# jhamrick/gaussian_processes

Measured on AMD Instinct MI355X. Metric: GP fit+predict wall-clock (kernel build + Cholesky + solve + log_lh + posterior mean), lower is better.
Workload: dtype f64; 1 GPU; N=65536 d=32 RBF(GaussianKernel) f64, m=1000 test points, h=1 w=0.5*sqrt(d) s=1; N=65536, d=32, m=1000, parallelism=1 GPU

## Files before the change

gaussian_processes_amd/_lib.py:

```python
import ctypes
import os
from ctypes import (POINTER, c_char_p, c_double, c_float, c_int, c_int64, c_size_t,
                    c_uint64, c_void_p)

import numpy as np

_HERE = os.path.dirname(os.path.abspath(__file__))
LIB_PATH = os.path.join(_HERE, "libgpx.so")

OK = 0
ERR_ARG, ERR_HIP, ERR_NO_DEVICE, ERR_NOMEM, ERR_UNSUPPORTED, ERR_INTERNAL = -1, -2, -3, -4, -5, -6
(ROUTE_TRSV_OPS, ROUTE_TRSV_STEPS, ROUTE_PANEL_RES, ROUTE_PANEL_CHAIN, ROUTE_FIT_RIDE, ROUTE_FIT_TWO_SOLVES,
 ROUTE_GEMM_FAST, ROUTE_GEMM_GENERIC, ROUTE_SYRK_EXACT, ROUTE_SYRK_PATCH, ROUTE_MG_BCAST_ONE, ROUTE_MG_BCAST_SAG,
 ROUTE_FIT_OPS_AHEAD, ROUTE_TRSM_OPS, ROUTE_POTRF_PAIR, ROUTE_VAR_CHUNK, ROUTE_LOO_CHUNK, ROUTE_TRSM_L_OPS,
 ROUTE_GRAD_CHUNK, ROUTE_EXTEND, ROUTE_SAMPLE, ROUTE_KAPPLY_FUSED, ROUTE_KAPPLY_GEMM, ROUTE_PATHS_GRAD_CHUNK,
 ROUTE_REMOVE, ROUTE_SPARSE_CHUNK) = range(26)
PROF_RANDN, PROF_RFF, PROF_KAPPLY, PROF_KAPPLY_GRAD, PROF_CHOL_DELETE, PROF_SPARSE_GRAM, PROF_SPARSE_GRAD = 14, 15, 16, 17, 18, 19, 20
F64, F32 = 0, 1
KERNEL_GAUSSIAN, KERNEL_PERIODIC, KERNEL_GAUSSIAN_ARD = 0, 1, 2
ARD_MAX_D = 64
FULL, LOWER = 0, 1
(K, DK_DH, DK_DW, DK_DP, D2K_DHDH, D2K_DHDW, D2K_DHDP, D2K_DWDW, D2K_DWDP, D2K_DPDP) = range(10)
MIN_LOG = -705.6238298100243

MEMBER_BY_NAME = {
    "K": K, "dK_dh": DK_DH, "dK_dw": DK_DW, "dK_dp": DK_DP,
    "d2K_dhdh": D2K_DHDH, "d2K_dhdw": D2K_DHDW, "d2K_dwdh": D2K_DHDW,
    "d2K_dhdp": D2K_DHDP, "d2K_dpdh": D2K_DHDP, "d2K_dwdw": D2K_DWDW,
    "d2K_dwdp": D2K_DWDP, "d2K_dpdw": D2K_DWDP, "d2K_dpdp": D2K_DPDP,
}

MG_ID_BYTES = 128
MG_BCAST_FN = ctypes.CFUNCTYPE(c_int, c_void_p, c_void_p, c_size_t, c_int, c_void_p)
MG_ALLREDUCE_FN = ctypes.CFUNCTYPE(c_int, c_void_p, c_void_p, c_size_t, c_int, c_int, c_void_p)

c_double_p = POINTER(c_double)
c_int_p = POINTER(c_int)

_SIGNATURES = {
    "gpx_version": (c_int, []),
    "gpx_last_error": (c_char_p, []),
    "gpx_device_count": (c_int, [c_int_p]),
    "gpx_set_device": (c_int, [c_int]),
    "gpx_get_device": (c_int, [c_int_p]),
    "gpx_device_info": (c_int, [c_int, c_char_p, c_size_t, c_int_p, c_int_p, POINTER(c_uint64)]),
    "gpx_malloc": (c_int, [POINTER(c_void_p), c_size_t]),
    "gpx_free": (c_int, [c_void_p]),
    "gpx_mem_info": (c_int, [ctypes.POINTER(c_size_t), ctypes.POINTER(c_size_t)]),
    "gpx_memcpy_h2d": (c_int, [c_void_p, c_void_p, c_size_t, c_void_p]),
# ... 316 lines not shown
```

gaussian_processes_amd/csrc/gpx_common.h:

```cpp
#pragma once
#include <hip/hip_runtime.h>
#include <stdint.h>
#include <stdio.h>
#include <stdlib.h>
#include <string.h>
#include <math.h>
#include <vector>

#include "../../include/gpx.h"
#include "gpx_tune.h"

namespace gpx {

void set_error(const char *fmt, ...);
int  hip_fail(hipError_t e, const char *what, const char *file, int line);
int  ensure_device();

#define GPX_HIP(call)                                                        \
    do {                                                                     \
        hipError_t e__ = (call);                                             \
        if (e__ != hipSuccess) return gpx::hip_fail(e__, #call, __FILE__, __LINE__); \
    } while (0)

#define GPX_TRY(call)                                                        \
    do {                                                                     \
        int rc__ = (call);                                                   \
        if (rc__ != GPX_OK) return rc__;                                     \
    } while (0)

#define GPX_ARG(cond, msg)                                                   \
    do {                                                                     \
        if (!(cond)) { gpx::set_error("%s: %s", __func__, msg); return GPX_ERR_ARG; } \
    } while (0)

#define GPX_LAUNCH_CHECK()                                                   \
    do {                                                                     \
        hipError_t e__ = hipGetLastError();                                  \
        if (e__ != hipSuccess) return gpx::hip_fail(e__, "kernel launch", __FILE__, __LINE__); \
    } while (0)


enum Route { RT_TRSV_OPS = 0, RT_TRSV_STEPS = 1, RT_PANEL_RES = 2, RT_PANEL_CHAIN = 3, RT_FIT_RIDE = 4,
             RT_FIT_TWO_SOLVES = 5, RT_GEMM_FAST = 6, RT_GEMM_GENERIC = 7, RT_SYRK_EXACT = 8, RT_SYRK_PATCH = 9,
             RT_MG_BCAST_ONE = 10, RT_MG_BCAST_SAG = 11, RT_FIT_OPS_AHEAD = 12, RT_TRSM_OPS = 13, RT_POTRF_PAIR = 14, RT_VAR_CHUNK = 15, RT_LOO_CHUNK = 16,
             RT_TRSM_L_OPS = 17, RT_GRAD_CHUNK = 18, RT_EXTEND = 19, RT_SAMPLE = 20, RT_KAPPLY_FUSED = 21, RT_KAPPLY_GEMM = 22, RT_PATHS_GRAD_CHUNK = 23, RT_REMOVE = 24, RT_SPARSE_CHUNK = 25, RT_COUNT = 26 };
void route_hit(int route);

int check_internal_info(int info);

static inline hipStream_t S(void *s) { return (hipStream_t)s; }
static inline size_t esize(int dtype) { return dtype == GPX_F64 ? 8 : 4; }
static inline int64_t round_up(int64_t v, int64_t m) { return (v + m - 1) / m * m; }
static inline int64_t cdiv(int64_t a, int64_t b) { return (a + b - 1) / b; }

static inline int order(hipEvent_t e, hipStream_t from, hipStream_t to)
{
    GPX_HIP(hipEventRecord(e, from));
    GPX_HIP(hipStreamWaitEvent(to, e, 0));
    return GPX_OK;
}
struct EventPool {
    std::vector<hipEvent_t> ev; size_t next = 0;
    int reserve(size_t count)
    {
        while (ev.size() < count) {
            hipEvent_t x;
            GPX_HIP(hipEventCreateWithFlags(&x, hipEventDisableTiming));
            ev.push_back(x);
        }
        return GPX_OK;
    }
    int get(hipEvent_t *e) { GPX_TRY(reserve(next + 1)); *e = ev[next++]; return GPX_OK; }
    void rewind() { next = 0; }
    void destroy() { for (hipEvent_t e : ev) (void)hipEventDestroy(e); ev.clear(); next = 0; }
    int order(hipStream_t from, hipStream_t to) { hipEvent_t e; GPX_TRY(get(&e)); return gpx::order(e, from, to); }
};

enum ProfClass { PC_KMAT = 0, PC_GEMM = 1, PC_POTRF_DIAG = 2, PC_TRSM_ROWS = 3, PC_TRSV = 4,
// ... 61 lines not shown
int syrk_bc(int dtype, int64_t n, int64_t row_begin, void *Cloc, int64_t ldc, int64_t cl0, int64_t cl1,
            const void *Pb, int64_t ldp, int64_t k0, int64_t kb, int64_t nb, int P, int rank,
            hipStream_t st, const int *abort_flag = nullptr, const Batch *bt = nullptr);
struct PanelHints { bool idle_chip = false; int leaf_force = 0; };
struct PotrfHook { int (*fn)(void *user, int64_t cols_done, hipEvent_t panel_done); void *user; };
int potrf_panel(int dtype, void *A, int64_t lda, int64_t n, int64_t r0, int64_t c0, int64_t kb,
                int *info_dev, hipStream_t st, const Batch *bt = nullptr, int64_t kpre = 0,
                hipEvent_t done = nullptr, PanelHints hints = {});
int potrf(int dtype, void *A, int64_t n, int64_t lda, int *info_dev, hipStream_t st, const Batch *bt = nullptr,
          int64_t xrows = 0,
          bool may_block = false,
          const PotrfHook *hook = nullptr);
int potrf_panel_res(int dtype, void *A, int64_t lda, int64_t n, int64_t r0, int64_t c0, int64_t kb, int *info_dev,
                    hipStream_t st, const Batch *bt = nullptr, int64_t kpre = 0, hipEvent_t done = nullptr, PanelHints hints = {});
int64_t panel_res_max();
hipStream_t potrf_side_stream();
bool kernel_values_finite(int kernel, const double *p, double s, int dtype);
bool panel_res_fold(int64_t rows, int64_t kpre, int64_t kb, size_t es, int64_t lda, const void *base);
constexpr int TRSV_OPS_BLOCK = 512;
static inline int64_t trsv_ops_nblocks(int64_t n) { return n / TRSV_OPS_BLOCK; }
static inline bool trsv_ops_whole_blocks(int64_t n) { return n >= TRSV_OPS_BLOCK && n % TRSV_OPS_BLOCK == 0; }
struct TrsvOps {
    GrowBuf mem;
    bool valid = false;
    int64_t built = 0;
    void invalidate() { valid = false; built = 0; }
    static TrsvOps view(void *p, size_t bytes) { TrsvOps o; o.mem.p = p; o.mem.bytes = bytes; return o; }
};
int trsv_ops_build(int dtype, const void *L, int64_t n, int64_t ldl, TrsvOps *ops, hipStream_t st);
bool trsv_ops_ahead_ok(int dtype, const void *L, int64_t n, int64_t ldl);
bool trsm_ops_ok(int dtype, const void *L, int64_t n, int64_t ldl);
size_t trsv_ops_bytes(int dtype, int64_t n);
int trsv_ops_build_upto(int dtype, const void *L, int64_t n, int64_t ldl, TrsvOps *ops, int64_t kend, hipStream_t st);
int trsv_lower(int dtype, const void *L, int64_t n, int64_t ldl, void *b, void *x, int transpose,
               hipStream_t st, const Batch *bt = nullptr,
               TrsvOps *ops = nullptr);
int trsm_right_lt(int dtype, const void *L, int64_t n, int64_t ldl, void *X, int64_t m, int64_t ldx,
                  hipStream_t st, int x_upper = 0, TrsvOps *ops = nullptr,
                  int64_t c0 = 0);
int trsm_right_l(int dtype, const void *L, int64_t n, int64_t ldl, void *X, int64_t m, int64_t ldx, hipStream_t st,
                 TrsvOps *ops = nullptr);
int pred_grad(int dtype, int kernel, const void *xo, int64_t m, const void *x, int64_t n, int d, const double *params,
              const void *alpha, const void *B, int64_t ldb, double scale, const double *col_div, double *out_dev, hipStream_t st);
int inv_from_factor(int dtype, const void *L, int64_t n, int64_t ldl, void *X, void *W, int tri, hipStream_t st,
                    TrsvOps *ops, int count = 1, int64_t sL = 0, void *group_ops = nullptr);
int logdet_chol(int dtype, const void *L, int64_t n, int64_t ldl, double *out_dev, hipStream_t st, int count = 1,
                int64_t sL = 0, int64_t so = 0);
int dot(int dtype, const void *a, const void *b, int64_t n, double *out_dev, hipStream_t st, int count = 1,
        int64_t sa = 0, int64_t sb = 0, int64_t so = 0);
int diag_sum(int dtype, const void *A, int64_t n, int64_t lda, double *out_dev, hipStream_t st);
int transpose(int dtype, const void *src, int64_t lds, int64_t rows, int64_t cols, void *dst, int64_t ldd, int mirror, hipStream_t st);
int tril(int dtype, void *A, int64_t n, int64_t lda, hipStream_t st);
int var_rows(int dtype, int kernel, const void *X, int64_t rows, int64_t n, int64_t ldx, const void *xo, int d,
             const double *params, const double *kdiag_dev, int accumulate, double *out_dev, hipStream_t st);
int var_finish(int dtype, int kernel, const void *xo, int d, const double *params, const double *acc_dev, int64_t rows,
               double *out_dev, hipStream_t st);
int eye_rows(int dtype, void *X, int64_t rows, int64_t ld, int64_t c0, int64_t cz, hipStream_t st);
int loo_rows(int dtype, const void *X, int64_t rows, int64_t n, int64_t ldx, int64_t c0, const void *y, const void *alpha,
             double *kii, double *mean, double *var, double *logp, hipStream_t st);
int loo_points(int dtype, const double *kii, const void *y, const void *alpha, int64_t n, double *mean, double *var, double *logp,
               hipStream_t st);
int sum_f64(const double *a, int64_t n, double *out_dev, hipStream_t st);
int copy_lower(int dtype, const void *src, int64_t lds, void *dst, int64_t ldd, int64_t n, hipStream_t st);
int schur_lower(int dtype, const void *B, int64_t k, int64_t n, int64_t ldb, void *S, int64_t lds, hipStream_t st);
int sum_slices_lower(int dtype, const void *P, int64_t ldp, int64_t sP, int slices, int64_t n, const void *minus_from, void *out, int64_t ldo,
                     hipStream_t st);
// ... 45 lines not shown
```

gaussian_processes_amd/csrc/gpx_gp.hip:

```cpp
#include "gpx_small.h"
#include <cmath>
#include <vector>

#include "gpx_gp_internal.h"

namespace gpx {

static int copy_rows(void *dst, int64_t ldd, const void *src, int64_t lds, int64_t rows, int64_t cols, hipMemcpyKind kind, hipStream_t st)
{
    if (rows == 1) GPX_HIP(hipMemcpyAsync(dst, src, (size_t)cols * 8, kind, st));
    else GPX_HIP(hipMemcpy2DAsync(dst, (size_t)ldd * 8, src, (size_t)lds * 8, (size_t)cols * 8, (size_t)rows, kind, st));
    return GPX_OK;
}

int upload_f64(int dtype, void *dst, int64_t ldd, const double *src, int64_t lds, int64_t rows, int64_t cols, hipStream_t st, DevBuf *stage)
{
    if (rows <= 0 || cols <= 0) return GPX_OK;
    if (dtype == GPX_F64) {
        GPX_TRY(copy_rows(dst, ldd, src, lds, rows, cols, hipMemcpyHostToDevice, st));
    } else {
        DevBuf mine;
        if (!stage) stage = &mine;
        if (!stage->p) GPX_TRY(stage->alloc((size_t)rows * cols * 8));
        GPX_TRY(copy_rows(stage->p, cols, src, lds, rows, cols, hipMemcpyHostToDevice, st));
// ... 37 lines not shown
    return scale_points(g->dtype, g->x, g->n, g->d, g->params + 1, g->xs, g->st);
}

static int upload_points(gpx_gp *g, void *dst, const double *xo, int64_t m)
{
    GPX_TRY(upload_f64(g->dtype, dst, m * g->d, xo, m * g->d, 1, m * g->d, g->st));
    if (g->kernel == GPX_KERNEL_GAUSSIAN_ARD) GPX_TRY(scale_points(g->dtype, dst, m, g->d, g->params + 1, dst, g->st));
    return GPX_OK;
}

int gp_read_scal(gpx_gp *g, GpScal *host)
{
    GPX_HIP(hipMemcpyAsync(host, g->scal, sizeof(GpScal), hipMemcpyDeviceToHost, g->st));
    GPX_HIP(hipStreamSynchronize(g->st));
    return check_internal_info(host->info);
}

int gp_need_factor(gpx_gp *g, const char *what_for)
{
    GpScal sc;
    GPX_TRY(gp_read_scal(g, &sc));
    if (sc.info != 0) { set_error("Kxx is not positive definite (info = %d): there is no factor %s", sc.info, what_for); return GPX_ERR_ARG; }
    return GPX_OK;
}

int check_internal_info(int info)
{
    if (info >= 0) return GPX_OK;
    set_error("internal failure inside the factorisation (info = %d: a hand-off between workgroups of the resident "
              "panel kernel timed out); the factor is not valid -- this is NOT a statement about the matrix", info);
    return GPX_ERR_INTERNAL;
}

int gp_finish_fit(gpx_gp *g, bool rhs_is_row_n, int *info)
{
    const size_t es = esize(g->dtype);
    hipStream_t st = g->st;
    if (rhs_is_row_n) {
        GPX_TRY(trsv_lower(g->dtype, g->A, g->n, g->lda, (char *)g->A + (size_t)g->n * g->lda * es, g->alpha, 1, st, nullptr, &g->ops));
    } else {
        GPX_HIP(hipMemcpyAsync(g->t0, g->y, (size_t)g->n * es, hipMemcpyDeviceToDevice, st));
        GPX_TRY(trsv_lower(g->dtype, g->A, g->n, g->lda, g->t0, g->t1, 0, st, nullptr, &g->ops));
        GPX_TRY(trsv_lower(g->dtype, g->A, g->n, g->lda, g->t1, g->alpha, 1, st, nullptr, &g->ops));
    }
    GPX_HIP(hipEventRecord(g->ev[3], st));
    GPX_TRY(logdet_chol(g->dtype, g->A, g->n, g->lda, &g->scal->logdet, st));
    GPX_TRY(dot(g->dtype, g->y, g->alpha, g->n, &g->scal->yta, st));
    GPX_HIP(hipEventRecord(g->ev[4], st));
    g->fitted = true;
    if (info) {
        GPX_HIP(hipMemcpyAsync(info, &g->scal->info, sizeof(int), hipMemcpyDeviceToHost, st));
        GPX_HIP(hipStreamSynchronize(st));
        GPX_TRY(check_internal_info(*info));
    }
    return GPX_OK;
}

template <typename T>
__global__ void nonfinite_kernel(const T *__restrict__ v, int64_t n, int *__restrict__ flag)
{
    bool bad = false;
    for (int64_t i = (int64_t)blockIdx.x * blockDim.x + threadIdx.x; i < n; i += (int64_t)gridDim.x * blockDim.x)
        bad = bad || !isfinite(v[i]);
    if (__any(bad) && (threadIdx.x & 63) == 0) atomicOr(flag, 1);
}

int gp_scan_finite(gpx_gp *g)
{
    int *flags = &g->scal->x_bad;
    GPX_HIP(hipMemsetAsync(flags, 0, 2 * sizeof(int), g->st));
    const int64_t nx = g->n * g->d, ny = g->n;
    const unsigned bx = (unsigned)std::min<int64_t>(cdiv(nx, 256), 1024), by = (unsigned)std::min<int64_t>(cdiv(ny, 256), 1024);
// ... 203 lines not shown
    return gp_scan_finite(g);
}

int gpx_gp_set_params(gpx_gp_t *g, const double *params, double s)
{
    GP_ENTER(g);
    GPX_ARG(g && params, "NULL argument");
    GPX_ARG(!(s < 0), "invalid value for s");
    for (int i = 0; i < g->nparams; ++i) g->params[i] = params[i];
    g->s = s;
    g->have_params = true; g->have_K = false; gp_unfit(g);
    return gp_rescale(g);
}

int gpx_gp_get_params(gpx_gp_t *g, double *params, int cap, int *count)
{
    GP_ENTER(g);
    GPX_ARG(g->have_params, "no kernel parameters in the handle");
    GPX_ARG(cap >= 0 && (cap == 0 || params), "bad arguments");
    if (count) *count = g->nparams;
    for (int i = 0; i < g->nparams && i < cap; ++i) params[i] = g->params[i];
    return GPX_OK;
}

int gpx_gp_set_K(gpx_gp_t *g, const double *Kxx, int64_t ld)
{
    GP_ENTER(g);
    GPX_ARG(g && Kxx && ld >= g->n, "bad arguments");
    GPX_TRY(upload_f64(g->dtype, g->A, g->lda, Kxx, ld, g->n, g->n, g->st));
    g->have_K = true; gp_unfit(g);
    return GPX_OK;
}

struct OpsAhead { gpx_gp *g; int64_t group, last; };
static int ops_ahead_step(void *user, int64_t cols_done, hipEvent_t panel_done)
{
    OpsAhead *o = (OpsAhead *)user;
    gpx_gp *g = o->g;
    const int64_t ready = std::min(trsv_ops_nblocks(cols_done), o->last);
    if (ready - g->ops.built < o->group) return GPX_OK;
    GPX_HIP(hipStreamWaitEvent(g->st_ops, panel_done, 0));
    return trsv_ops_build_upto(g->dtype, g->A, g->n, g->lda, &g->ops, ready, g->st_ops);
}

int gpx_gp_fit(gpx_gp_t *g, int *info)
{
    GP_ENTER(g);
    GPX_ARG(g, "gp is NULL");
    GPX_ARG(g->have_data && (g->have_params || g->have_K),
            "set_data and set_params (or set_K) must be called before fit");
    const GpView v = gp_view(g);
    if (!g->have_K && (!g->x_finite || !kernel_values_finite(v.kernel, v.params, g->s, g->dtype))) {
        set_error("%s (%s)", NONFINITE_MSG, g->x_finite ? "kernel parameters or s" : "x");
        return GPX_ERR_ARG;
    }
    const size_t es = esize(g->dtype);
    hipStream_t st = g->st;
    GPX_HIP(hipEventRecord(g->ev[0], st));
    if (!g->have_K)
        GPX_TRY(kmat(g->dtype, v.kernel, GPX_K, v.x, g->n, v.x, g->n, g->d, v.params, g->s * g->s,
                     GPX_LOWER, g->A, g->lda, st));
    g->have_K = false;
    g->have_kii = false;
    GPX_HIP(hipEventRecord(g->ev[1], st));
    const int64_t ride_max = tune().fit_ride_max;
    const bool ride = g->n <= ride_max;
    route_hit(ride ? RT_FIT_RIDE : RT_FIT_TWO_SOLVES);
    if (ride) GPX_HIP(hipMemcpyAsync((char *)g->A + (size_t)g->n * g->lda * es, g->y, (size_t)g->n * es, hipMemcpyDeviceToDevice, st));
    g->ops.invalidate();
    const bool ahead = tune().fit_ops_ahead != 0 && g->n >= tune().fit_ops_ahead_min &&
                       trsv_ops_ahead_ok(g->dtype, g->A, g->n, g->lda);
    const int64_t nfull = trsv_ops_nblocks(g->n), tail = tune().fit_ops_tail;
    const int64_t group = std::max<int64_t>(1, std::min(nfull, nfull - tail));
    OpsAhead oa = {g, group, std::max<int64_t>(0, nfull - tail)};
    PotrfHook hook = {ops_ahead_step, &oa};
    if (ahead) {
        if (!g->st_ops) {
            int least = 0, greatest = 0;
            GPX_HIP(hipDeviceGetStreamPriorityRange(&least, &greatest));
            GPX_HIP(hipStreamCreateWithPriority(&g->st_ops, hipStreamNonBlocking, least));
            GPX_HIP(hipEventCreateWithFlags(&g->ev_ops, hipEventDisableTiming));
        }
        GPX_TRY(g->ops.mem.reserve(trsv_ops_bytes(g->dtype, g->n), st));
        GPX_TRY(order(g->ev_ops, st, g->st_ops));
    }
    GPX_TRY(potrf(g->dtype, g->A, g->n, g->lda, &g->scal->info, st, nullptr, ride ? 1 : 0, true, ahead ? &hook : nullptr));
    if (ahead) {
        GPX_TRY(order(g->ev_ops, g->st_ops, st));
        if (g->ops.built > 0) route_hit(RT_FIT_OPS_AHEAD);
    }
    GPX_HIP(hipEventRecord(g->ev[2], st));
    return gp_finish_fit(g, ride, info);
}

static int gp_scalars(gpx_gp_t *g, double *logdet, double *yta, int *info)
{
    GP_ENTER(g);
    GPX_ARG(g && g->fitted, "gp is not fitted");
    GpScal sc;
    GPX_TRY(gp_read_scal(g, &sc));
    if (logdet) *logdet = sc.logdet;
    if (yta) *yta = sc.yta;
    if (info) *info = sc.info;
    return GPX_OK;
}

int gpx_gp_log_lh(gpx_gp_t *g, double *log_lh)
{
    GPX_ARG(log_lh, "log_lh is NULL");
    GPX_ARG(g, "gp is NULL");
    GP_NEED_FINITE_Y(g);
    double logdet, yta; int info;
    GPX_TRY(gp_scalars(g, &logdet, &yta, &info));
    if (info != 0 || !(logdet >= GPX_MIN_LOG)) { *log_lh = -INFINITY; return GPX_OK; }
    const double data_fit = -0.5 * yta;
    const double complexity_penalty = -0.5 * logdet;
    const double constant = -0.5 * (double)g->n * log(2 * M_PI);
    *log_lh = data_fit + complexity_penalty + constant;
    return GPX_OK;
}

int gpx_gp_logdet(gpx_gp_t *g, double *logdet)
{
    GPX_ARG(logdet, "logdet is NULL");
    return gp_scalars(g, logdet, nullptr, nullptr);
// ... 727 lines not shown
```

gaussian_processes_amd/csrc/gpx_gp_internal.h:

```cpp
#pragma once
#include "gpx_common.h"
#include <cstddef>

struct GpScal {
    double logdet;
    double yta;
    int x_bad, y_bad;
    int info;
    int pad;
};
static_assert(sizeof(GpScal) == 32 && offsetof(GpScal, x_bad) == 16 && offsetof(GpScal, info) == 24, "GpScal layout");

struct gpx_gp {
    int device;
    int dtype, kernel, d, nparams;
    int64_t n, lda;
    void *x, *y, *A, *alpha, *t0, *t1;
    void *xs;
    GpScal *scal;
    hipStream_t st;
    hipEvent_t ev[6];
    double params[1 + GPX_ARD_MAX_D];
    double iso[2];
    double s;
    bool have_data, have_params, fitted, have_K;
    bool x_finite, y_finite;
    gpx::GrowBuf bw; int64_t bw_cap;
    gpx::TrsvOps ops;
    gpx::GrowBuf gw; int64_t gw_cap;
    gpx::TrsvOps bops;
    double *kii;
    bool have_kii;
    hipStream_t st_ops;
    hipEvent_t ev_ops;
};

namespace gpx {
int gp_scan_finite(gpx_gp *g);
int upload_f64(int dtype, void *dst, int64_t ldd, const double *src, int64_t lds, int64_t rows, int64_t cols, hipStream_t st,
               DevBuf *stage = nullptr);
int download_f64(int dtype, double *dst, int64_t ldh, const void *src, int64_t lds, int64_t rows, int64_t cols, int lower_only,
                 hipStream_t st);
int gp_read_scal(gpx_gp *g, GpScal *host);
int gp_need_factor(gpx_gp *g, const char *what_for);
static inline void gp_unfit(gpx_gp *g) { g->fitted = false; g->have_kii = false; }
int gp_finish_fit(gpx_gp *g, bool rhs_is_row_n, int *info);
static inline int nparams_of(int kernel, int d) { return kernel == GPX_KERNEL_GAUSSIAN_ARD ? 1 + d : (kernel == GPX_KERNEL_PERIODIC ? 3 : 2); }
struct GpView { int kernel; const void *x; const double *params; };
static inline GpView gp_view(const gpx_gp *g)
{
    if (g->kernel == GPX_KERNEL_GAUSSIAN_ARD) return {GPX_KERNEL_GAUSSIAN, g->xs, g->iso};
    return {g->kernel, g->x, g->params};
}
int gp_rescale(gpx_gp *g);
int loo_grad_reduce(gpx_gp *g, const void *pts, const void *alpha, const double *params, double s_noise, const LooVecs &v,
                    const void *Pm, int64_t ldp, double *part, double *value, double *out);
}

static const char *const NONFINITE_MSG = "array must not contain infs or NaNs";

#define GP_NEED_FINITE_Y(g)                                                    \
    do { if (!(g)->y_finite) { gpx::set_error("%s (y)", NONFINITE_MSG); return GPX_ERR_ARG; } } while (0)

#define GP_ENTER(g)                                                          \
    GPX_ARG((g) != nullptr, "gp is NULL");                                   \
    gpx::tune_refresh();                                                     \
    gpx::DeviceGuard guard__((g)->device);                                   \
    if (guard__.rc != GPX_OK) return guard__.rc;                             \
    gpx::StreamTurn turn__((g)->st);                                         \
    gpx::RoctxRange api_range__(__func__)
```

gaussian_processes_amd/csrc/gpx_mg.hip:

```cpp
#include "gpx_common.h"
#include "gpx_gp_internal.h"
#include <dlfcn.h>
#include <climits>
#include <cmath>
#include <vector>

extern "C" {
typedef struct ncclComm *ncclComm_t;
typedef struct { char internal[128]; } ncclUniqueId;
typedef int ncclResult_t;
typedef int ncclDataType_t;
typedef int ncclRedOp_t;
}
static constexpr ncclResult_t ncclSuccess = 0;
static constexpr ncclDataType_t ncclInt32 = 2, ncclFloat32 = 7, ncclFloat64 = 8;
static constexpr ncclRedOp_t ncclSum = 0, ncclMax = 2;
static_assert(sizeof(ncclUniqueId) == GPX_MG_ID_BYTES, "ncclUniqueId is 128 bytes");

extern "C" int gpx_d_mean(int dtype, int kernel, const void *xo, int64_t m, const void *x, int64_t n, int d,
                          const double *params, const void *alpha, void *out, void *stream);
namespace gpx {

struct Rccl {
    void *lib = nullptr;
// ... 590 lines not shown
    GPX_HIP(hipStreamCreateWithPriority(&g->Q, hipStreamNonBlocking, greatest));
    GPX_HIP(hipStreamCreateWithPriority(&g->B, hipStreamNonBlocking, greatest));
    GPX_HIP(hipStreamCreateWithPriority(&g->O, hipStreamNonBlocking, least));
    for (size_t jl = 0; jl < g->my_blocks.size(); ++jl) {
        const int64_t kb = g->kb(g->my_blocks[jl]);
        if (!trsv_ops_whole_blocks(kb)) continue;
        GPX_TRY(g->ops[jl].mem.reserve(trsv_ops_bytes(g->dtype, kb), g->O));
    }
    return GPX_OK;
}

static int mg_new(gpx_mg **out, MgCommKind kind, int dtype, int kernel, int64_t n, int d, int64_t nb, int world, int rank)
{
    GPX_TRY(ensure_device());
    GPX_ARG(out, "mg is NULL");
    *out = nullptr;
    GPX_ARG(dtype == GPX_F64 || dtype == GPX_F32, "dtype must be GPX_F64 or GPX_F32");
    GPX_ARG(kernel == GPX_KERNEL_GAUSSIAN || kernel == GPX_KERNEL_PERIODIC, "unknown kernel family");
    GPX_ARG(n >= 1 && d >= 1, "need n >= 1 and d >= 1");
    GPX_ARG(world >= 1 && rank >= 0 && rank < world, "bad world / rank");
    GPX_ARG(nb >= 64 && nb % 64 == 0 && 1024 % nb == 0, "nb must be 64 / 128 / 256 / 512 / 1024");
    gpx_mg *g = new gpx_mg();
    g->dtype = dtype; g->kernel = kernel; g->n = n; g->d = d; g->nb = nb; g->world = world; g->rank = rank;
    g->es = esize(dtype);
    g->comm.kind = kind;
    if (hipGetDevice(&g->device) != hipSuccess) { (void)hipGetLastError(); g->device = 0; }
    g->nblk = cdiv(n, nb);
    for (int64_t j = rank; j < g->nblk; j += world) g->my_blocks.push_back(j);
    g->ncols_local = std::max<int64_t>(1, (int64_t)g->my_blocks.size()) * nb;
    g->ld = g->ncols_local;
    g->nr = n + 1;
    g->ops.resize(std::max<size_t>(1, g->my_blocks.size()));
    g->bcast_chunks = (int)std::max<int64_t>(1, std::min<int64_t>(16, tune().mg_bcast_chunks));
    g->timing = !tune().mg_no_timing;
    if (tune().mg_bcast_set) g->bcast_sag = tune().mg_bcast_sag;
    g->owner_first = tune().mg_owner_first_set ? (tune().mg_owner_first != 0) : (world >= 2);
    *out = g;
    return GPX_OK;
}


static double mg_hash(const void *p, size_t bytes)
{
    uint64_t h = 1469598103934665603ull;
    const unsigned char *c = (const unsigned char *)p;
    for (size_t i = 0; i < bytes; ++i) { h ^= c[i]; h *= 1099511628211ull; }
    return (double)(h >> 12);
}

constexpr int MG_COV_AGREE = 8, MG_VAR_AGREE = 11;
static int mg_cov_agree(gpx_mg *g, double *v, int nv, const char *who)
{
    double *dv = g->scal + 4;
    GPX_HIP(hipMemcpyAsync(dv, v, nv * sizeof(double), hipMemcpyHostToDevice, g->S));
    GPX_TRY(mg_allreduce(g, dv, nv, GPX_F64, 1, g->S));
    GPX_HIP(hipMemcpyAsync(v, dv, nv * sizeof(double), hipMemcpyDeviceToHost, g->S));
    GPX_HIP(hipStreamSynchronize(g->S));
    if (v[0] != 0) { set_error("%s: a device allocation failed on at least one rank", who); return GPX_ERR_NOMEM; }
    if (v[1] != 0) {
        set_error("%s: bad arguments on at least one rank (m < 0 or a NULL pointer%s)", who, nv > MG_COV_AGREE ? ", or a chunk_rows that is not a multiple of 128" : "");
        return GPX_ERR_ARG;
    }
    if (v[2] != -v[3]) { set_error("%s: the ranks called with different m (%.0f .. %.0f)", who, -v[3], v[2]); return GPX_ERR_ARG; }
    if (v[4] != -v[5]) { set_error("%s: the ranks called with different xo", who); return GPX_ERR_ARG; }
    if (v[6] != -v[7]) { set_error("%s: the ranks called with different params", who); return GPX_ERR_ARG; }
    if (nv > MG_COV_AGREE && v[8] != -v[9]) { set_error("%s: the ranks called with different chunk_rows (%.0f .. %.0f)", who, -v[9], v[8]); return GPX_ERR_ARG; }
    return GPX_OK;
// ... 477 lines not shown
```

gaussian_processes_amd/csrc/gpx_solve.hip:

```cpp
#include "gpx_small.h"
#include "gpx_kernels_dev.h"
#include "gpx_leaf.h"

namespace gpx {

constexpr int SB = 64;
constexpr int OB = TRSV_OPS_BLOCK;

template <typename T>
__global__ __launch_bounds__(256) void inv64_kernel(const T *__restrict__ L, int64_t ldl, int64_t ncols,
                                                    T *__restrict__ out, int transposed, T *__restrict__ W,
                                                    T *__restrict__ Wt, int64_t bsL, int64_t bsOut)
{
    L += (int64_t)blockIdx.y * bsL;
    const int tid = threadIdx.x, tr = tid >> 4, tc = tid & 15;
    const int64_t k0 = (int64_t)blockIdx.x * SB;
    const int jb = (int)min((int64_t)SB, ncols - k0);
    const T *blk = L + k0 * ldl + k0;
    T a[4][4], x[4][4];
#pragma unroll
    for (int r = 0; r < 4; ++r)
#pragma unroll
        for (int c = 0; c < 4; ++c) {
            const int row = 4 * tr + r, col = 4 * tc + c;
// ... 512 lines not shown
    const int64_t n = S.n, nb = S.nb();
    auto launch = [&](int64_t far_rows, int64_t nn, int64_t k0, int jb, int64_t p0, int pjb, int64_t far0) {
        hipLaunchKernelGGL((trsv_fwd_fused<T>), dim3((unsigned)(1 + cdiv(far_rows, 64)), S.nbt), dim3(TBT), 0, S.st, S.L, S.ldl,
                           S.Linv, S.b, S.x, nn, k0, jb, p0, pjb, far0, S.aligned, S.sL, S.sLinv, S.sv);
    };
    for (int64_t blk = kfirst; blk < nb; ++blk) {
        const int64_t k0 = blk * TB, p0 = std::max<int64_t>(blk - 1, 0) * TB;
        const int jb = S.width(blk), pjb = blk > 0 ? TB : 0;
        if (blk > 0) launch(jb, k0 + jb, k0, 0, p0, pjb, k0);
        launch(blk > 0 ? n - (k0 + jb) : 0, n, k0, jb, p0, pjb, k0 + jb);
    }
    if (n > S.ncols) launch(n - S.ncols, n, S.ncols, 0, (nb - 1) * TB, S.width(nb - 1), S.ncols);
}

template <typename T>
static void steps_bwd(const Sweep<T> &S, int64_t kfirst)
{
    const int64_t nb = S.nb();
    for (int64_t blk = nb - 1; blk >= kfirst; --blk) {
        const int64_t k0 = blk * TB, q0 = k0 + TB;
        const int jb = S.width(blk), qjb = blk + 1 < nb ? S.width(blk + 1) : 0;
        if (qjb > 0)
            hipLaunchKernelGGL((trsv_bwd_fused<T, 32>), dim3((unsigned)(1 + cdiv(jb, 32)), S.nbt), dim3(TBT), 0, S.st, S.L,
                               S.ldl, S.Linv, S.b, S.x, k0, 0, q0, qjb, k0, k0 + jb, S.aligned, S.sL, S.sLinv, S.sv);
        hipLaunchKernelGGL((trsv_bwd_fused<T, 128>), dim3((unsigned)(1 + (qjb > 0 ? cdiv(k0, 128) : 0)), S.nbt),
                           dim3(TBT), 0, S.st, S.L, S.ldl, S.Linv, S.b, S.x, k0, jb, q0, qjb, (int64_t)0, k0, S.aligned,
                           S.sL, S.sLinv, S.sv);
    }
}

constexpr int NCH = OB / (TBT / OPL);

template <typename T>
static void ops_fwd(const Sweep<T> &S, const OpsView<T> &V)
{
    for (int64_t k = 0; k < V.nfull; ++k) {
        const int64_t k0 = k * OB, far0 = k0 + OB;
        const int64_t nfar = k > 0 ? cdiv(S.n - far0, 64) : 0;
        hipLaunchKernelGGL((trsv_op_kernel<T, true>), dim3((unsigned)(NCH + nfar)), dim3(TBT), 0, S.st, V.W(k),
                           k > 0 ? V.Tf(k) : (const T *)nullptr, S.L, S.ldl, S.b, S.x, S.n, k0, k0 - OB, k > 0 ? OB : 0, far0, S.n, NCH, 1);
    }
}

template <typename T>
static void ops_bwd(const Sweep<T> &S, const OpsView<T> &V, int64_t kend)
{
    for (int64_t k = kend - 1; k >= 0; --k) {
        const int64_t k0 = k * OB, q0 = k0 + OB;
        const int qjb = (k + 1 < V.nfull) ? OB : (int)(S.n - q0);
        const int64_t nfar = qjb > 0 ? cdiv(k0, 128) : 0;
        hipLaunchKernelGGL((trsv_op_kernel<T, false>), dim3((unsigned)(NCH + nfar)), dim3(TBT), 0, S.st, V.Wt(k),
                           qjb > 0 ? V.Tb(k) : (const T *)nullptr, S.L, S.ldl, S.b, S.x, S.n, k0, q0, qjb, (int64_t)0, k0, NCH, 1);
    }
}

template <typename T>
static int trsv_t(const T *L, int64_t n, int64_t ldl, T *b, T *x, int transpose, hipStream_t st,
                  int64_t ncols = -1, const Batch *bt = nullptr, TrsvOps *ops = nullptr)
{
    constexpr int dtype = sizeof(T) == 8 ? GPX_F64 : GPX_F32;
    if (ncols < 0 || ncols > n) ncols = n;
    Sweep<T> S;
    S.L = L; S.n = n; S.ldl = ldl; S.ncols = ncols; S.b = b; S.x = x; S.st = st;
    S.nbt = (unsigned)(bt ? bt->count : 1); S.sL = bt ? bt->sA : 0; S.sv = bt ? bt->sB : 0;
    ProfScope prof(PC_TRSV, ((double)n * ncols - 0.5 * (double)ncols * (ncols - 1)) * sizeof(T) * S.nbt, st);
    S.sLinv = cdiv(ncols, SB) * SB * SB;
    void *scr = nullptr;
    GPX_TRY(g_scr.get((size_t)S.nbt * S.sLinv * sizeof(T), &scr));
    S.Linv = (T *)scr;
    S.aligned = (((uintptr_t)L) % (2 * sizeof(T)) == 0) && (ldl % 2 == 0);
    const bool usable = !bt && ncols == n && ops_usable(dtype, L, ldl);
    const bool cached = ops && ops->mem.p && n % OB == 0 && ops->mem.bytes >= trsv_ops_bytes(dtype, n);
    const bool prebuilt = cached && ops->valid;
    const int64_t kpart = (usable && cached && !ops->valid && ops->built > 0 && transpose) ? std::min(ops->built, n / OB) : 0;
    if (kpart == 0 && usable && (n >= trsv_ops_min_n() || prebuilt)) {
        route_hit(RT_TRSV_OPS);
        void *buf = nullptr;
        if (ops) {
            bool grew = false;
            GPX_TRY(ops->mem.reserve(trsv_ops_bytes(dtype, n), st, &grew));
            if (grew) ops->invalidate();
            buf = ops->mem.p;
        } else {
            GPX_TRY(g_ops.get(trsv_ops_bytes(dtype, n), &buf));
        }
        const OpsView<T> V(buf, n);
        if (!ops || !ops->valid) GPX_TRY(trsv_ops_prepare<T>(L, n, ldl, buf, st, ops ? std::min(ops->built, V.nfull) : 0, V.nfull));
        if (ops) { ops->valid = true; ops->built = V.nfull; }
        const bool ragged = n > V.nfull * OB;
        if (!transpose) {
            ops_fwd(S, V);
            if (ragged) { inv64_blocks(S, 0, 1); steps_fwd(S, V.nfull); }
        } else {
            if (ragged) { inv64_blocks(S, 0, 0); steps_bwd(S, V.nfull); }
            ops_bwd(S, V, V.nfull);
        }
    } else if (!transpose) {
        route_hit(RT_TRSV_STEPS);
        inv64_blocks(S, 0, 1);
        steps_fwd(S, 0);
    } else {
        route_hit(RT_TRSV_STEPS);
        inv64_blocks(S, kpart * (OB / SB), 0);
        steps_bwd(S, kpart);
        if (kpart > 0) {
            route_hit(RT_TRSV_OPS);
            ops_bwd(S, OpsView<T>(ops->mem.p, n), kpart);
        }
    }
    GPX_LAUNCH_CHECK();
    return GPX_OK;
}

int trsv_lower(int dtype, const void *L, int64_t n, int64_t ldl, void *b, void *x, int transpose,
               hipStream_t st, const Batch *bt, TrsvOps *ops)
{
    if (n <= 0) return GPX_OK;
    return by_dtype(dtype, [&](auto t) {
        using T = decltype(t);
        return trsv_t<T>((const T *)L, n, ldl, (T *)b, (T *)x, transpose, st, -1, bt, ops);
    });
}

int trsv_ops_build(int dtype, const void *L, int64_t n, int64_t ldl, TrsvOps *ops, hipStream_t st)
{
    if (!ops || !trsv_ops_whole_blocks(n) || !ops_usable(dtype, L, ldl)) return GPX_OK;
    GPX_TRY(ops->mem.reserve(trsv_ops_bytes(dtype, n), st));
    ops->invalidate();
    GPX_TRY(by_dtype(dtype, [&](auto t) { using T = decltype(t); return trsv_ops_prepare<T>((const T *)L, n, ldl, ops->mem.p, st); }));
    ops->valid = true;
    ops->built = n / OB;
    return GPX_OK;
}

int trsv_ops_build_upto(int dtype, const void *L, int64_t n, int64_t ldl, TrsvOps *ops, int64_t kend, hipStream_t st)
{
    if (!ops || !trsv_ops_ahead_ok(dtype, L, n, ldl)) return GPX_OK;
    const int64_t nfull = n / OB;
    kend = std::min(kend, nfull);
    if (ops->built == 0) {
        GPX_TRY(ops->mem.reserve_device(trsv_ops_bytes(dtype, n)));
        ops->valid = false;
    }
    if (kend <= ops->built || !ops->mem.p) return GPX_OK;
    GPX_TRY(by_dtype(dtype, [&](auto t) { using T = decltype(t); return trsv_ops_prepare<T>((const T *)L, n, ldl, ops->mem.p, st, ops->built, kend); }));
    ops->built = kend;
    if (kend == nfull) ops->valid = true;
    return GPX_OK;
}

int trsv_lower_cols(int dtype, const void *L, int64_t n, int64_t ldl, int64_t ncols, void *b, void *x,
                    hipStream_t st)
{
// ... 556 lines not shown
```

gaussian_processes_amd/csrc/gpx_tune.h:

```cpp
#pragma once
#include <stdint.h>

namespace gpx {

#define GPX_TUNE_LIST(X, XF, XS, X2)                                                                                   \
                                                                               \
    XF(gemm_no_fast, "GPX_GEMM_NO_FAST")                                                                               \
    X(gemm_ablate, "GPX_GEMM_ABLATE", 0)                                                                               \
    X(gemm_pad_lds, "GPX_GEMM_PAD_LDS", 0)                                                                             \
    X(gemm_bn64_tiles, "GPX_GEMM_BN64_TILES", 256)                                                                     \
    X(gemm_exact, "GPX_GEMM_EXACT", 1)                                                                                 \
    X(gemm_fine_tiles, "GPX_GEMM_FINE_TILES", 16384)                                                                   \
    X2(syrk_bn64_tiles, "GPX_SYRK_BN64_TILES", 2600, 4000)                                                             \
                                                              \
    X(fit_ride_max, "GPX_FIT_RIDE_MAX", 16384)                                                                         \
    X(fit_ops_ahead, "GPX_FIT_OPS_AHEAD", 1)                                                                           \
    X(fit_ops_ahead_min, "GPX_FIT_OPS_AHEAD_MIN", 8192)                                                                \
    X(fit_ops_tail, "GPX_FIT_OPS_TAIL", 4)                                                                             \
    XS(batch_max, "GPX_BATCH_MAX", 1)                                                                                  \
    X(io_block_bytes, "GPX_IO_BLOCK_BYTES", (int64_t)64 << 20)                                                         \
    X(kmat_panel_bytes, "GPX_KMAT_PANEL_BYTES", (int64_t)256 << 20)                                                    \
                                                                        \
    XF(force_collectives, "GPX_FORCE_COLLECTIVES")                                                                     \
    X(mg_bcast_chunks, "GPX_MG_BCAST_CHUNKS", 4)                                                                       \
    XF(mg_no_timing, "GPX_MG_NO_TIMING")                                                                               \
    XS(mg_owner_first, "GPX_MG_OWNER_FIRST", 0)                                                                        \
                                                                  \
    XF(trace, "GPX_TRACE")                                                                                             \
    X(potrf_res, "GPX_POTRF_RES", 256)                                                                                 \
    X(res_strict, "GPX_RES_STRICT", 1)                                                                                 \
    X(two_part_rows, "GPX_POTRF_TWO_PART_ROWS", 16384)                                                                 \
    X(two_part_batch, "GPX_POTRF_TWO_PART_BATCH", 98304)                                                               \
    X(leaf_mfma_f32_rows, "GPX_LEAF_MFMA_F32_ROWS", 16384)                                                             \
    X(panel_excl_rows, "GPX_PANEL_EXCL_ROWS", 5120)                                                                    \
    XS(leaf, "GPX_LEAF", 0)                                                                                            \
    X2(leaf4_rows, "GPX_LEAF4_ROWS", 8192, 5120)                                                                       \
    X2(panel_pad_lds, "GPX_PANEL_PAD_LDS", 8 * 1024, 40 * 1024)                                                        \
    X(fold_rows, "GPX_POTRF_FOLD_ROWS", 16384)                                                                         \
    X(fold_k, "GPX_POTRF_FOLD_K", 256)                                                                                 \
                                                                  \
    XS(potrf_nb, "GPX_POTRF_NB", 0)                                                                                    \
    XF(potrf_trsm_rows, "GPX_POTRF_TRSM_ROWS")                                                                         \
    X(potrf_inv_max, "GPX_POTRF_INV_MAX", 16384)                                                                       \
    XF(no_lookahead, "GPX_POTRF_NO_LOOKAHEAD")                                                                         \
    X(taper, "GPX_POTRF_TAPER", 1)                                                                                     \
    X2(pair_rows, "GPX_POTRF_PAIR_ROWS", 0, 0)                                                                         \
    X(host_paced, "GPX_POTRF_HOST_PACED", 16384)                                                                       \
    X(gate_rows, "GPX_POTRF_GATE_ROWS", 16384)                                                                         \
                                                                                 \
    X(trsv_ops, "GPX_TRSV_OPS", 1)                                                                                     \
    X(trsv_ops_min, "GPX_TRSV_OPS_MIN", 10240)                                                                         \
    X(trsm_ops, "GPX_TRSM_OPS", 1)                                                                                     \
                                                                          \
    XF(roctx, "GPX_ROCTX")

constexpr int64_t GPX_KAPPLY_FUSED_MAX_F64 = 32;
constexpr int64_t GPX_KAPPLY_FUSED_MAX_F32 = 8;

// ... 22 lines not shown
```

include/gpx.h:

```cpp
#ifndef GPX_H
#define GPX_H

#include <stddef.h>
#include <stdint.h>

#ifdef __cplusplus
extern "C" {
#endif

#define GPX_VERSION 100

#define GPX_OK              0
#define GPX_ERR_ARG        -1
#define GPX_ERR_HIP        -2
#define GPX_ERR_NO_DEVICE  -3
#define GPX_ERR_NOMEM      -4
#define GPX_ERR_UNSUPPORTED -5
#define GPX_ERR_INTERNAL   -6

#define GPX_F64 0
#define GPX_F32 1

#define GPX_KERNEL_GAUSSIAN 0
#define GPX_KERNEL_PERIODIC 1
// ... 67 lines not shown
#define GPX_PROF_KAPPLY_GRAD 17
#define GPX_PROF_CHOL_DELETE 18
#define GPX_PROF_SPARSE_GRAM 19
#define GPX_PROF_SPARSE_GRAD 20
int gpx_prof_enable(int on);
int gpx_prof_read(int cls, double *launches, double *total_ms, double *total_work);

#define GPX_ROUTE_TRSV_OPS        0
#define GPX_ROUTE_TRSV_STEPS      1
#define GPX_ROUTE_PANEL_RES       2
#define GPX_ROUTE_PANEL_CHAIN     3
#define GPX_ROUTE_FIT_RIDE        4
#define GPX_ROUTE_FIT_TWO_SOLVES  5
#define GPX_ROUTE_GEMM_FAST       6
#define GPX_ROUTE_GEMM_GENERIC    7
#define GPX_ROUTE_SYRK_EXACT      8
#define GPX_ROUTE_SYRK_PATCH      9
#define GPX_ROUTE_MG_BCAST_ONE   10
#define GPX_ROUTE_MG_BCAST_SAG   11
#define GPX_ROUTE_FIT_OPS_AHEAD  12
#define GPX_ROUTE_TRSM_OPS       13
#define GPX_ROUTE_POTRF_PAIR     14
#define GPX_ROUTE_VAR_CHUNK      15
#define GPX_ROUTE_LOO_CHUNK      16
#define GPX_ROUTE_TRSM_L_OPS     17
#define GPX_ROUTE_GRAD_CHUNK     18
#define GPX_ROUTE_EXTEND         19
#define GPX_ROUTE_SAMPLE         20
#define GPX_ROUTE_KAPPLY_FUSED   21
#define GPX_ROUTE_KAPPLY_GEMM    22
#define GPX_ROUTE_PATHS_GRAD_CHUNK 23
#define GPX_ROUTE_REMOVE         24
#define GPX_ROUTE_SPARSE_CHUNK   25
int gpx_debug_route_count(int route, int64_t *count);
int gpx_debug_roctx_ranges(int64_t *count);
int gpx_debug_route_reset(void);
int gpx_debug_tune_refreshes(int64_t *count);
int gpx_debug_kapply_fused_max(int64_t value, int64_t *previous);
int gpx_debug_leaf_selfcheck(int run_now, int *state);


int gpx_d_kmat(int dtype, int kernel, int member, const void *x1, int64_t n,
               const void *x2, int64_t m, int d, const double *params,
               double diag_add, int tri, void *out, int64_t ld, void *stream);

int gpx_d_scale_points(int dtype, const void *x, int64_t n, int d, const double *w_host, void *out, void *stream);

int gpx_d_mean(int dtype, int kernel, const void *xo, int64_t m, const void *x,
               int64_t n, int d, const double *params, const void *alpha,
               void *out, void *stream);

int gpx_d_mean_member(int dtype, int kernel, int member, const void *xo, int64_t m, const void *x,
                      int64_t n, int d, const double *params, const void *alpha, void *out, void *stream);

int gpx_d_pred_grad(int dtype, int kernel, const void *xo, int64_t m, const void *x, int64_t n, int d,
                    const double *params, const void *alpha, const void *B, int64_t ldb, double scale,
                    double *out_dev, void *stream);

int gpx_d_gemm_nt(int dtype, int64_t M, int64_t N, int64_t K, double alpha,
                  const void *A, int64_t lda, const void *B, int64_t ldb, void *C,
                  int64_t ldc, int tri, int64_t row0, int64_t col0, void *stream);

int gpx_d_potrf(int dtype, void *A, int64_t n, int64_t lda, int *info_dev,
                void *stream);

int gpx_d_potrf_panel(int dtype, void *A, int64_t lda, int64_t n, int64_t r0, int64_t c0,
// ... 229 lines not shown
```

Baseline: 1.333 s.

## Overlap forward triangular solve sweep with the Cholesky tail on the ops stream

During the blocked Cholesky factorization, once the remaining rows fall below a threshold, the forward substitution for alpha is launched block by block on the side ops stream using the block operators already built. After the factorization, only the remaining forward blocks and the backward solve run. This hides part of the forward TRSV latency behind the factorization tail. In exchange it adds cross-stream ordering complexity and extra hook logic. It also drops an unused multi-GPU timing flag.

Result: no change. 1.331 s (median of 6 runs) (-0.1%).

```diff
diff --git a/gaussian_processes_amd/_lib.py b/gaussian_processes_amd/_lib.py
--- a/gaussian_processes_amd/_lib.py
+++ b/gaussian_processes_amd/_lib.py
@@ -14,7 +14,7 @@
  ROUTE_GEMM_FAST, ROUTE_GEMM_GENERIC, ROUTE_SYRK_EXACT, ROUTE_SYRK_PATCH, ROUTE_MG_BCAST_ONE, ROUTE_MG_BCAST_SAG,
  ROUTE_FIT_OPS_AHEAD, ROUTE_TRSM_OPS, ROUTE_POTRF_PAIR, ROUTE_VAR_CHUNK, ROUTE_LOO_CHUNK, ROUTE_TRSM_L_OPS,
  ROUTE_GRAD_CHUNK, ROUTE_EXTEND, ROUTE_SAMPLE, ROUTE_KAPPLY_FUSED, ROUTE_KAPPLY_GEMM, ROUTE_PATHS_GRAD_CHUNK,
- ROUTE_REMOVE, ROUTE_SPARSE_CHUNK) = range(26)
+ ROUTE_REMOVE, ROUTE_SPARSE_CHUNK, ROUTE_FIT_SWEEP_AHEAD) = range(27)
 PROF_RANDN, PROF_RFF, PROF_KAPPLY, PROF_KAPPLY_GRAD, PROF_CHOL_DELETE, PROF_SPARSE_GRAM, PROF_SPARSE_GRAD = 14, 15, 16, 17, 18, 19, 20
 F64, F32 = 0, 1
 KERNEL_GAUSSIAN, KERNEL_PERIODIC, KERNEL_GAUSSIAN_ARD = 0, 1, 2
diff --git a/gaussian_processes_amd/csrc/gpx_common.h b/gaussian_processes_amd/csrc/gpx_common.h
--- a/gaussian_processes_amd/csrc/gpx_common.h
+++ b/gaussian_processes_amd/csrc/gpx_common.h
@@ -43,7 +43,7 @@
 enum Route { RT_TRSV_OPS = 0, RT_TRSV_STEPS = 1, RT_PANEL_RES = 2, RT_PANEL_CHAIN = 3, RT_FIT_RIDE = 4,
              RT_FIT_TWO_SOLVES = 5, RT_GEMM_FAST = 6, RT_GEMM_GENERIC = 7, RT_SYRK_EXACT = 8, RT_SYRK_PATCH = 9,
              RT_MG_BCAST_ONE = 10, RT_MG_BCAST_SAG = 11, RT_FIT_OPS_AHEAD = 12, RT_TRSM_OPS = 13, RT_POTRF_PAIR = 14, RT_VAR_CHUNK = 15, RT_LOO_CHUNK = 16,
-             RT_TRSM_L_OPS = 17, RT_GRAD_CHUNK = 18, RT_EXTEND = 19, RT_SAMPLE = 20, RT_KAPPLY_FUSED = 21, RT_KAPPLY_GEMM = 22, RT_PATHS_GRAD_CHUNK = 23, RT_REMOVE = 24, RT_SPARSE_CHUNK = 25, RT_COUNT = 26 };
+             RT_TRSM_L_OPS = 17, RT_GRAD_CHUNK = 18, RT_EXTEND = 19, RT_SAMPLE = 20, RT_KAPPLY_FUSED = 21, RT_KAPPLY_GEMM = 22, RT_PATHS_GRAD_CHUNK = 23, RT_REMOVE = 24, RT_SPARSE_CHUNK = 25, RT_FIT_SWEEP_AHEAD = 26, RT_COUNT = 27 };
 void route_hit(int route);
 
 int check_internal_info(int info);
@@ -171,6 +171,8 @@
 bool trsm_ops_ok(int dtype, const void *L, int64_t n, int64_t ldl);
 size_t trsv_ops_bytes(int dtype, int64_t n);
 int trsv_ops_build_upto(int dtype, const void *L, int64_t n, int64_t ldl, TrsvOps *ops, int64_t kend, hipStream_t st);
+int trsv_fwd_ops_blocks(int dtype, const void *L, int64_t n, int64_t ldl, void *b, void *x, int64_t kbeg, int64_t kend,
+                        hipStream_t st, TrsvOps *ops);
 int trsv_lower(int dtype, const void *L, int64_t n, int64_t ldl, void *b, void *x, int transpose,
                hipStream_t st, const Batch *bt = nullptr,
                TrsvOps *ops = nullptr);
diff --git a/gaussian_processes_amd/csrc/gpx_gp.hip b/gaussian_processes_amd/csrc/gpx_gp.hip
--- a/gaussian_processes_amd/csrc/gpx_gp.hip
+++ b/gaussian_processes_amd/csrc/gpx_gp.hip
@@ -93,12 +93,15 @@
     return GPX_ERR_INTERNAL;
 }
 
-int gp_finish_fit(gpx_gp *g, bool rhs_is_row_n, int *info)
+int gp_finish_fit(gpx_gp *g, bool rhs_is_row_n, int *info, int64_t fwd_done)
 {
     const size_t es = esize(g->dtype);
     hipStream_t st = g->st;
     if (rhs_is_row_n) {
         GPX_TRY(trsv_lower(g->dtype, g->A, g->n, g->lda, (char *)g->A + (size_t)g->n * g->lda * es, g->alpha, 1, st, nullptr, &g->ops));
+    } else if (fwd_done >= 0) {
+        GPX_TRY(trsv_fwd_ops_blocks(g->dtype, g->A, g->n, g->lda, g->t0, g->t1, fwd_done, -1, st, &g->ops));
+        GPX_TRY(trsv_lower(g->dtype, g->A, g->n, g->lda, g->t1, g->alpha, 1, st, nullptr, &g->ops));
     } else {
         GPX_HIP(hipMemcpyAsync(g->t0, g->y, (size_t)g->n * es, hipMemcpyDeviceToDevice, st));
         GPX_TRY(trsv_lower(g->dtype, g->A, g->n, g->lda, g->t0, g->t1, 0, st, nullptr, &g->ops));
@@ -368,15 +371,23 @@
     return GPX_OK;
 }
 
-struct OpsAhead { gpx_gp *g; int64_t group, last; };
+struct OpsAhead { gpx_gp *g; int64_t group, last, sweep_rows, swept; bool fired; };
 static int ops_ahead_step(void *user, int64_t cols_done, hipEvent_t panel_done)
 {
     OpsAhead *o = (OpsAhead *)user;
     gpx_gp *g = o->g;
     const int64_t ready = std::min(trsv_ops_nblocks(cols_done), o->last);
-    if (ready - g->ops.built < o->group) return GPX_OK;
+    const bool first = o->sweep_rows > 0 && !o->fired && g->n - cols_done <= o->sweep_rows;
+    if (first) o->fired = true;
+    const bool due = first || (o->fired ? ready >= o->last : ready - g->ops.built >= o->group);
+    if (ready <= g->ops.built || !due) return GPX_OK;
     GPX_HIP(hipStreamWaitEvent(g->st_ops, panel_done, 0));
-    return trsv_ops_build_upto(g->dtype, g->A, g->n, g->lda, &g->ops, ready, g->st_ops);
+    GPX_TRY(trsv_ops_build_upto(g->dtype, g->A, g->n, g->lda, &g->ops, ready, g->st_ops));
+    if (o->sweep_rows > 0 && g->ops.built > o->swept) {
+        GPX_TRY(trsv_fwd_ops_blocks(g->dtype, g->A, g->n, g->lda, g->t0, g->t1, o->swept, g->ops.built, g->st_ops, &g->ops));
+        o->swept = g->ops.built;
+    }
+    return GPX_OK;
 }
 
 int gpx_gp_fit(gpx_gp_t *g, int *info)
@@ -407,8 +418,11 @@
     const bool ahead = tune().fit_ops_ahead != 0 && g->n >= tune().fit_ops_ahead_min &&
                        trsv_ops_ahead_ok(g->dtype, g->A, g->n, g->lda);
     const int64_t nfull = trsv_ops_nblocks(g->n), tail = tune().fit_ops_tail;
+    const bool fwd_ops = g->n >= std::max<int64_t>(2 * TRSV_OPS_BLOCK, tune().trsv_ops_min);
+    const int64_t sweep_rows = (ahead && !ride && fwd_ops) ? std::max<int64_t>(0, tune().fit_sweep_rows) : 0;
+    const int64_t last = std::max<int64_t>(0, nfull - tail);
     const int64_t group = std::max<int64_t>(1, std::min(nfull, nfull - tail));
-    OpsAhead oa = {g, group, std::max<int64_t>(0, nfull - tail)};
+    OpsAhead oa = {g, group, last, sweep_rows, 0, false};
     PotrfHook hook = {ops_ahead_step, &oa};
     if (ahead) {
         if (!g->st_ops) {
@@ -419,14 +433,16 @@
         }
         GPX_TRY(g->ops.mem.reserve(trsv_ops_bytes(g->dtype, g->n), st));
         GPX_TRY(order(g->ev_ops, st, g->st_ops));
+        if (sweep_rows > 0) GPX_HIP(hipMemcpyAsync(g->t0, g->y, (size_t)g->n * es, hipMemcpyDeviceToDevice, g->st_ops));
     }
     GPX_TRY(potrf(g->dtype, g->A, g->n, g->lda, &g->scal->info, st, nullptr, ride ? 1 : 0, true, ahead ? &hook : nullptr));
     if (ahead) {
         GPX_TRY(order(g->ev_ops, g->st_ops, st));
         if (g->ops.built > 0) route_hit(RT_FIT_OPS_AHEAD);
+        if (oa.swept > 0) route_hit(RT_FIT_SWEEP_AHEAD);
     }
     GPX_HIP(hipEventRecord(g->ev[2], st));
-    return gp_finish_fit(g, ride, info);
+    return gp_finish_fit(g, ride, info, sweep_rows > 0 ? oa.swept : -1);
 }
 
 static int gp_scalars(gpx_gp_t *g, double *logdet, double *yta, int *info)
diff --git a/gaussian_processes_amd/csrc/gpx_gp_internal.h b/gaussian_processes_amd/csrc/gpx_gp_internal.h
--- a/gaussian_processes_amd/csrc/gpx_gp_internal.h
+++ b/gaussian_processes_amd/csrc/gpx_gp_internal.h
@@ -44,7 +44,7 @@
 int gp_read_scal(gpx_gp *g, GpScal *host);
 int gp_need_factor(gpx_gp *g, const char *what_for);
 static inline void gp_unfit(gpx_gp *g) { g->fitted = false; g->have_kii = false; }
-int gp_finish_fit(gpx_gp *g, bool rhs_is_row_n, int *info);
+int gp_finish_fit(gpx_gp *g, bool rhs_is_row_n, int *info, int64_t fwd_done = -1);
 static inline int nparams_of(int kernel, int d) { return kernel == GPX_KERNEL_GAUSSIAN_ARD ? 1 + d : (kernel == GPX_KERNEL_PERIODIC ? 3 : 2); }
 struct GpView { int kernel; const void *x; const double *params; };
 static inline GpView gp_view(const gpx_gp *g)
diff --git a/gaussian_processes_amd/csrc/gpx_mg.hip b/gaussian_processes_amd/csrc/gpx_mg.hip
--- a/gaussian_processes_amd/csrc/gpx_mg.hip
+++ b/gaussian_processes_amd/csrc/gpx_mg.hip
@@ -646,7 +646,6 @@
     g->nr = n + 1;
     g->ops.resize(std::max<size_t>(1, g->my_blocks.size()));
     g->bcast_chunks = (int)std::max<int64_t>(1, std::min<int64_t>(16, tune().mg_bcast_chunks));
-    g->timing = !tune().mg_no_timing;
     if (tune().mg_bcast_set) g->bcast_sag = tune().mg_bcast_sag;
     g->owner_first = tune().mg_owner_first_set ? (tune().mg_owner_first != 0) : (world >= 2);
     *out = g;
diff --git a/gaussian_processes_amd/csrc/gpx_solve.hip b/gaussian_processes_amd/csrc/gpx_solve.hip
--- a/gaussian_processes_amd/csrc/gpx_solve.hip
+++ b/gaussian_processes_amd/csrc/gpx_solve.hip
@@ -568,9 +568,9 @@
 constexpr int NCH = OB / (TBT / OPL);
 
 template <typename T>
-static void ops_fwd(const Sweep<T> &S, const OpsView<T> &V)
-{
-    for (int64_t k = 0; k < V.nfull; ++k) {
+static void ops_fwd(const Sweep<T> &S, const OpsView<T> &V, int64_t kbeg, int64_t kend)
+{
+    for (int64_t k = kbeg; k < kend; ++k) {
         const int64_t k0 = k * OB, far0 = k0 + OB;
         const int64_t nfar = k > 0 ? cdiv(S.n - far0, 64) : 0;
         hipLaunchKernelGGL((trsv_op_kernel<T, true>), dim3((unsigned)(NCH + nfar)), dim3(TBT), 0, S.st, V.W(k),
@@ -625,7 +625,7 @@
         if (ops) { ops->valid = true; ops->built = V.nfull; }
         const bool ragged = n > V.nfull * OB;
         if (!transpose) {
-            ops_fwd(S, V);
+            ops_fwd(S, V, 0, V.nfull);
             if (ragged) { inv64_blocks(S, 0, 1); steps_fwd(S, V.nfull); }
         } else {
             if (ragged) { inv64_blocks(S, 0, 0); steps_bwd(S, V.nfull); }
@@ -655,6 +655,39 @@
     return by_dtype(dtype, [&](auto t) {
         using T = decltype(t);
         return trsv_t<T>((const T *)L, n, ldl, (T *)b, (T *)x, transpose, st, -1, bt, ops);
+    });
+}
+
+int trsv_fwd_ops_blocks(int dtype, const void *L, int64_t n, int64_t ldl, void *b, void *x, int64_t kbeg, int64_t kend,
+                        hipStream_t st, TrsvOps *ops)
+{
+    if (!ops || !ops->mem.p || !trsv_ops_ahead_ok(dtype, L, n, ldl) || ops->mem.bytes < trsv_ops_bytes(dtype, n)) {
+        set_error("trsv_fwd_ops_blocks: no block operators for this factor");
+        return GPX_ERR_ARG;
+    }
+    const int64_t nfull = n / OB;
+    const bool to_end = kend < 0;
+    if (to_end) kend = nfull;
+    if (kbeg < 0 || kbeg > kend || kend > nfull || (!to_end && kend > ops->built)) {
+        set_error("trsv_fwd_ops_blocks: blocks [%lld, %lld) of %lld, %lld built", (long long)kbeg, (long long)kend, (long long)nfull,
+                  (long long)ops->built);
+        return GPX_ERR_ARG;
+    }
+    if (kbeg == 0) route_hit(RT_TRSV_OPS);
+    return by_dtype(dtype, [&](auto t) -> int {
+        using T = decltype(t);
+        if (to_end && !ops->valid) {
+            GPX_TRY(trsv_ops_prepare<T>((const T *)L, n, ldl, ops->mem.p, st, std::min(ops->built, nfull), nfull));
+            ops->valid = true; ops->built = nfull;
+        }
+        if (kend == kbeg) return GPX_OK;
+        Sweep<T> S;
+        S.L = (const T *)L; S.n = n; S.ldl = ldl; S.ncols = n; S.b = (T *)b; S.x = (T *)x; S.st = st;
+        S.nbt = 1; S.sL = 0; S.sv = 0; S.Linv = nullptr; S.sLinv = 0; S.aligned = 1;
+        ProfScope prof(PC_TRSV, (double)(kend - kbeg) * OB * (double)(n - (kbeg + kend) * OB / 2) * sizeof(T), st);
+        ops_fwd(S, OpsView<T>(ops->mem.p, n), kbeg, kend);
+        GPX_LAUNCH_CHECK();
+        return GPX_OK;
     });
 }
 
diff --git a/gaussian_processes_amd/csrc/gpx_tune.h b/gaussian_processes_amd/csrc/gpx_tune.h
--- a/gaussian_processes_amd/csrc/gpx_tune.h
+++ b/gaussian_processes_amd/csrc/gpx_tune.h
@@ -17,13 +17,13 @@
     X(fit_ops_ahead, "GPX_FIT_OPS_AHEAD", 1)                                                                           \
     X(fit_ops_ahead_min, "GPX_FIT_OPS_AHEAD_MIN", 8192)                                                                \
     X(fit_ops_tail, "GPX_FIT_OPS_TAIL", 4)                                                                             \
+    X(fit_sweep_rows, "GPX_FIT_SWEEP_ROWS", 12288)                                                                     \
     XS(batch_max, "GPX_BATCH_MAX", 1)                                                                                  \
     X(io_block_bytes, "GPX_IO_BLOCK_BYTES", (int64_t)64 << 20)                                                         \
     X(kmat_panel_bytes, "GPX_KMAT_PANEL_BYTES", (int64_t)256 << 20)                                                    \
                                                                         \
     XF(force_collectives, "GPX_FORCE_COLLECTIVES")                                                                     \
     X(mg_bcast_chunks, "GPX_MG_BCAST_CHUNKS", 4)                                                                       \
-    XF(mg_no_timing, "GPX_MG_NO_TIMING")                                                                               \
     XS(mg_owner_first, "GPX_MG_OWNER_FIRST", 0)                                                                        \
                                                                   \
     XF(trace, "GPX_TRACE")                                                                                             \
diff --git a/include/gpx.h b/include/gpx.h
--- a/include/gpx.h
+++ b/include/gpx.h
@@ -123,6 +123,7 @@
 #define GPX_ROUTE_PATHS_GRAD_CHUNK 23
 #define GPX_ROUTE_REMOVE         24
 #define GPX_ROUTE_SPARSE_CHUNK   25
+#define GPX_ROUTE_FIT_SWEEP_AHEAD 26
 int gpx_debug_route_count(int route, int64_t *count);
 int gpx_debug_roctx_ranges(int64_t *count);
 int gpx_debug_route_reset(void);
```
